# marbl/Mash

Measured on AMD Instinct MI355X. Metric: pairwise Mash distances/sec (s=1000), higher is better.
Workload: dtype u64; 1 GPU; mash triangle all-vs-all, 100000 clustered synthetic sketches, k=21 s=1000, 4999950000 pairs/step, per-table job (index build + discover + fill + merge each step), row-block sharded x1; parallelism=rowblock1, rccl_ranks=0

## Files before the change

### mash_amd/csrc/compare_dense.hip

```cpp
#ifdef MG_HIP_EMU
#include "hipemu.h"
#else
#include <hip/hip_runtime.h>
#define MG_DYN_SHARED(T, name)                                   \
    extern __shared__ __align__(16) unsigned char name##_raw[]; \
    T *name = reinterpret_cast<T *>(name##_raw)
#endif
#include <stdint.h>

#include <cstdlib>

#ifndef MG_HIP_EMU
#include <rocprim/device/device_radix_sort.hpp>
#include <rocprim/device/device_select.hpp>
#include <rocprim/iterator/counting_iterator.hpp>
#endif

#include "compare_internal.h"

namespace mg {

#ifndef MG_HIP_EMU
__global__ __launch_bounds__(256) void dn_neighbor_kernel(const uint64_t *hashes, uint64_t stride, const uint32_t *cnt, uint32_t n,
                                                          uint8_t *link)
// ... 126 lines not shown
{
    if (E == 0) return hipSuccess;
    hipError_t e = hipMemsetAsync(cnt, 0, DN_SUBLISTS * 4, stream);
    if (e == hipSuccess) e = hipMemsetAsync(total, 0, 8, stream);
    if (e != hipSuccess) return e;
    hipLaunchKernelGGL(dn_leaders_kernel, dim3((E + 255u) / 256u), dim3(256), 0, stream, sorted_rows, gs_of, gend, grp_of, groups, E, key, val, cap_sub,
                       cnt);
    e = hipGetLastError();
    if (e != hipSuccess) return e;
    return dense_join_leaders(key, val, cap_sub, key_out, val_out, cnt, off, total, stream);
}

hipError_t dense_join_leaders(const unsigned long long *key, const uint32_t *val, uint32_t cap_sub, unsigned long long *key_out, uint32_t *val_out,
                              const uint32_t *cnt, uint32_t *off, uint32_t *total, hipStream_t stream)
{
    hipLaunchKernelGGL(dn_sublists_scan_kernel, dim3(1), dim3(DN_SUBLISTS), 0, stream, cnt, cap_sub, off, total);
    hipLaunchKernelGGL(dn_sublists_copy_kernel, dim3(DN_SUBLISTS), dim3(256), 0, stream, key, val, cnt, (const uint32_t *)off, cap_sub, key_out, val_out);
    return hipGetLastError();
}

hipError_t dense_sort_universes(const unsigned long long *key, const uint32_t *val, uint32_t m, void *temp, size_t temp_bytes,
                                unsigned long long *key_sorted, uint32_t *ulist, uint32_t *upos, uint32_t *ustart, uint32_t *uend,
                                uint32_t group_bits, hipStream_t stream)
{
    if (m == 0) return hipSuccess;
    hipError_t e = rocprim::radix_sort_pairs(temp, temp_bytes, key, key_sorted, val, upos, (size_t)m, 0u, 32u + group_bits, stream);
    if (e != hipSuccess) return e;
    hipLaunchKernelGGL(dn_universe_split_kernel, dim3((m + 255u) / 256u), dim3(256), 0, stream, (const unsigned long long *)key_sorted, m, ulist,
                       ustart, uend);
    return hipGetLastError();
}

#endif

constexpr uint32_t DN_CX_MASK = 0x7FFFu, DN_CX_FLAG = 0x8000u;

template <uint32_t DN_EK>
__global__ __launch_bounds__(256) void dn_encode_kernel(const uint32_t *off, const uint32_t *code_img, uint32_t *pos_img, uint32_t rs,
                                                        const uint32_t *grp_of, const DenseGroup *groups, const uint32_t *ulist,
                                                        const uint32_t *upos, unsigned long long *gdata, uint32_t wstride, uint16_t *ext,
                                                        uint32_t xs, uint32_t n, uint32_t ul_in_lds)
{
    MG_DYN_SHARED(uint32_t, lds);
    const uint32_t bid = blockIdx.x;
    const uint32_t row = (bid & ~63u) | ((bid & 7u) << 3) | ((bid >> 3) & 7u);
    const uint32_t tid = threadIdx.x, lane = tid & 63u, wid = tid >> 6;
    if (row >= n) return;
    const uint32_t g = grp_of[row];
    if (g == 0xFFFFFFFFu) return;
    const DenseGroup G = groups[g];
    const uint32_t W = G.W, u = G.u;
    uint32_t *mask32 = lds, *hist = lds + 2u * W, *gap8 = hist + W + 1u, *ovf = gap8 + 16u * W, *pl32 = ovf + W, *scr = pl32 + 8u * W;
    uint32_t *ull = lds + 28u * wstride + 9u;
    for (uint32_t i = tid; i < 28u * W + 1u; i += 256u) lds[i] = 0;
    const uint32_t *ulg = ulist + G.ustart, *up = upos + G.ustart;
    if (ul_in_lds)
        for (uint32_t i = tid; i < u; i += 256u) ull[i] = ulg[i];
    const uint32_t *ul = ul_in_lds ? ull : ulg;
    __syncthreads();
    const uint32_t cnt = off[row + 1] - off[row];
    uint16_t *xrow = ext + (uint64_t)(G.xrow0 + (row - G.g0)) * xs;
    uint32_t nx = 0;
    if constexpr (DN_EK == 1) {
        for (uint32_t base = 0; base < cnt; base += 256u) {
            const uint32_t p = base + tid;
            uint32_t idx = 0;
// ... 493 lines not shown
{
    const uint32_t a = blockIdx.x;
    const uint64_t *src = hashes + (uint64_t)inv[a] * stride;
    uint64_t *dst = out + (uint64_t)a * stride;
    for (uint64_t p = threadIdx.x; p < stride; p += 256u) dst[p] = src[p];
}

hipError_t launch_dense_gather_rows(const uint64_t *hashes, uint64_t stride, const uint32_t *inv, uint32_t n, uint64_t *out, hipStream_t stream)
{
    if (n == 0) return hipSuccess;
    hipLaunchKernelGGL(cl_gather_rows_kernel, dim3(n), dim3(256), 0, stream, hashes, stride, inv, out);
    return hipGetLastError();
}

#endif

__global__ __launch_bounds__(256) void dn_group_rows_kernel(const DenseGroup *groups, uint32_t ng, uint32_t n, uint32_t *grp_of, uint4 *lead_rows)
{
    const uint32_t r = blockIdx.x * 256u + threadIdx.x;
    if (r >= n) return;
    uint32_t lo = 0, hi = ng;
    while (lo < hi) {
        const uint32_t mid = (lo + hi) >> 1;
        if (groups[mid].g0 <= r) lo = mid + 1u;
        else hi = mid;
    }
    uint32_t g = 0xFFFFFFFFu, g0 = 0, g1 = 0;
    if (lo > 0 && r < groups[lo - 1u].g1) {
        g = lo - 1u;
        g0 = groups[g].g0;
        g1 = groups[g].g1;
    }
    grp_of[r] = g;
    lead_rows[r] = make_uint4(g, g0, g1, 0u);
}

hipError_t launch_dense_group_rows(const DenseGroup *groups, uint32_t ng, uint32_t n, uint32_t *grp_of, uint32_t *lead_rows, hipStream_t stream)
{
    if (n == 0) return hipSuccess;
    hipLaunchKernelGGL(dn_group_rows_kernel, dim3((n + 255u) / 256u), dim3(256), 0, stream, groups, ng, n, grp_of, reinterpret_cast<uint4 *>(lead_rows));
    return hipGetLastError();
}

}
```

### mash_amd/csrc/compare_internal.h

```cpp
#pragma once
#ifdef MG_HIP_EMU
#include "hipemu.h"
#else
#include <hip/hip_runtime.h>
#endif
#include <stdint.h>

namespace mg {

struct MergedTile {
    uint32_t rows[32];
    uint32_t col0, col1;
};

struct CompareArgs {
    const uint64_t *row_hashes;
    const uint32_t *row_nhash;
    const uint64_t *col_hashes;
    const uint32_t *col_nhash;
    const uint32_t *row_pfx;
    const uint32_t *col_pfx;
    const MergedTile *mtiles;
    uint2 *out;
    uint64_t row_stride, col_stride;
// ... 137 lines not shown
    uint32_t g0, g1;
    uint32_t ustart, u;
    uint32_t W;
    uint32_t xrow0;
    uint64_t data_off;
};
struct DenseTile { uint32_t group, row0, cblk; };
#ifdef __HIPCC__
__host__ __device__
#endif
static inline uint64_t dense_block_planes(uint32_t W) { return 128ull * W + 64ull * (W + 1u); }
#ifdef __HIPCC__
__host__ __device__
#endif
static inline uint64_t dense_block_words(uint32_t W) { return dense_block_planes(W) + 512ull * W; }
struct DenseList {
    const uint32_t *row_base = nullptr, *row_cnt = nullptr;
    uint2 *rc = nullptr, *counts = nullptr;
    uint32_t row_first = 0;
};
hipError_t launch_dense_neighbors(const uint64_t *hashes, uint64_t stride, const uint32_t *cnt, uint32_t n, uint8_t *link,
                                  hipStream_t stream);
size_t dense_universe_temp_bytes(uint32_t cap);
uint32_t dense_sublists();
hipError_t dense_find_leaders(const uint32_t *sorted_rows, const uint32_t *gs_of, const uint32_t *gend, const uint32_t *grp_of,
                              const DenseGroup *groups, uint32_t E, unsigned long long *key, uint32_t *val, uint32_t cap_sub,
                              unsigned long long *key_out, uint32_t *val_out, uint32_t *cnt, uint32_t *off, uint32_t *total,
                              hipStream_t stream);
hipError_t dense_join_leaders(const unsigned long long *key, const uint32_t *val, uint32_t cap_sub, unsigned long long *key_out, uint32_t *val_out,
                              const uint32_t *cnt, uint32_t *off, uint32_t *total, hipStream_t stream);
hipError_t dense_sort_universes(const unsigned long long *key, const uint32_t *val, uint32_t m, void *temp, size_t temp_bytes,
                                unsigned long long *key_sorted, uint32_t *ulist, uint32_t *upos, uint32_t *ustart, uint32_t *uend,
                                uint32_t group_bits, hipStream_t stream);
hipError_t launch_dense_encode(const uint32_t *off, const uint32_t *code_img, uint32_t *pos_img, uint32_t rs, const uint32_t *grp_of,
                               const DenseGroup *groups, const uint32_t *ulist, const uint32_t *upos, unsigned long long *gdata,
                               uint16_t *ext, uint32_t xs, uint32_t n, uint32_t wmax, hipStream_t stream, int ul_mode = -1);
size_t dense_pairs_lds(uint32_t W, uint32_t rows);
uint32_t dense_rows_per_tile(uint64_t wave_rows);
uint32_t dense_max_words();
hipError_t launch_dense_pairs(const DenseTile *tiles, uint32_t ntiles, uint32_t rows_per_tile, const DenseGroup *groups,
                              const unsigned long long *gdata, bool use_lists, const uint16_t *ext, uint32_t xs,
                              uint32_t s, uint32_t wmax, uint32_t row_begin, uint32_t row_end, uint64_t out_base, const uint32_t *inv, uint2 *out,
                              hipStream_t stream, const DenseList *list = nullptr);
size_t dense_cluster_temp_bytes(uint32_t n);
hipError_t dense_cluster_rows(const uint64_t *hashes, uint64_t stride, const uint32_t *cnt, uint32_t n, void *temp, size_t temp_bytes,
                              unsigned long long *key_a, unsigned long long *key_b, uint32_t *row_a, uint32_t *row_b, uint32_t *lab_a,
                              uint32_t *lab_b, uint32_t *inv, uint32_t *label_sorted, hipStream_t stream, uint32_t split = 0);
hipError_t launch_dense_gather_rows(const uint64_t *hashes, uint64_t stride, const uint32_t *inv, uint32_t n, uint64_t *out, hipStream_t stream);
hipError_t launch_dense_group_rows(const DenseGroup *groups, uint32_t ng, uint32_t n, uint32_t *grp_of, uint32_t *lead_rows, hipStream_t stream);

struct JoinSide {
    const uint2 *grp = nullptr;
    const uint32_t *ent = nullptr;
    const uint32_t *goff = nullptr;
    const uint32_t *gend = nullptr;
    const uint32_t *thr = nullptr;
};
struct JoinArgs {
    JoinSide rows, cols;
    const uint32_t *row_cnt_off, *col_cnt_off;
    const uint32_t *rep, *col_rep;
    const uint32_t *inv;
    uint2 *out;
    uint64_t out_base;
    uint64_t ntiles;
    uint32_t ncols;
// ... 41 lines not shown
```

### mash_amd/csrc/host_index.cpp

```cpp
#include "host_internal.h"
#include "index_build.h"
#ifdef IX_PHASE_CLOCKS
namespace mg { void index_dump_clocks(); }
#endif
#include "sort_bits.h"

namespace {

const uint64_t kTilesLongestRun = 6144;
static const uint64_t kSplitMinRun = 128;

uint64_t longest_label_run(const uint32_t *lab_sorted, uint64_t n)
{
    if (!lab_sorted || n == 0) return 0;
    uint64_t run = 1, longest = 1;
    for (uint64_t a = 1; a < n; a++) {
        run = lab_sorted[a] == lab_sorted[a - 1] ? run + 1 : 1;
        longest = std::max(longest, run);
    }
    return longest;
}

struct Carve {
    unsigned char *base = nullptr;
    size_t at = 0;
    template <class T> T *take(size_t count)
    {
        const size_t from = (at + alignof(T) - 1) & ~(alignof(T) - 1);
        at = from + count * sizeof(T);
        return base ? reinterpret_cast<T *>(base + from) : nullptr;
    }
};

struct LeaderLists {
    DevBuf<unsigned long long> key, keyj;
    DevBuf<uint32_t> val, valj, cnt_sub, off_sub, nlead;
    uint32_t lists = mg::dense_sublists(), cap = 0, tot[2] = {0, 0};
    explicit LeaderLists(mg_ctx *c) : key(c), keyj(c), val(c), valj(c), cnt_sub(c), off_sub(c), nlead(c) {}

    hipError_t alloc(uint32_t room)
    {
        key.free(); val.free(); keyj.free(); valj.free();
        const uint64_t all = (uint64_t)lists * room;
        if (!(nlead.p && cnt_sub.p && off_sub.p) && (nlead.alloc(2) != hipSuccess || cnt_sub.alloc(lists) != hipSuccess || off_sub.alloc(lists) != hipSuccess))
            return hipErrorOutOfMemory;
        if (key.alloc(all) != hipSuccess || val.alloc(all) != hipSuccess || keyj.alloc(all) != hipSuccess || valj.alloc(all) != hipSuccess) return hipErrorOutOfMemory;
        cap = room;
        return hipSuccess;
    }
    hipError_t reset(hipStream_t st) { const hipError_t e = hipMemsetAsync(cnt_sub, 0, lists * 4, st); return e != hipSuccess ? e : hipMemsetAsync(nlead, 0, 8, st); }
    hipError_t join(hipStream_t st)
    {
        const hipError_t e = mg::dense_join_leaders(key, val, cap, keyj, valj, cnt_sub, off_sub, nlead, st);
        return e != hipSuccess ? e : hipMemcpyAsync(tot, nlead, 8, hipMemcpyDeviceToHost, st);
    }
    mg::IxLeaders view(const uint32_t *lead_rows) const { return mg::IxLeaders{lead_rows, key, val, cnt_sub, cap, lists}; }
    bool overflowed() const { return tot[1] > cap; }
};

struct SparseIndexBuild {
    mg_ctx *ctx;
    const mg_table *t;
    const uint32_t s;
    const bool clustered;
    const uint32_t split;
    mg_table::Sparse *sp;
    const uint64_t n;
    const std::chrono::steady_clock::time_point t_begin = std::chrono::steady_clock::now();
    bool stop = false;

    bool need_classes = false, dedup = true, want_dense = true, try_cluster = false, try_links = false;
    DevBuf<uint8_t> dc_cls, d_link;
    DevBuf<unsigned long long> dc_last, d_dig, d_dig_sorted, k_a, k_b;
    DevBuf<uint32_t> d_cnt, d_rows_sorted, d_flags, d_nflag, r_a, r_b, l_a, l_b, d_inv, d_lab;
    DevBuf<unsigned char> d_tmp_dup, d_tmp_cl;
    std::vector<uint8_t> hc_cls, link;
    std::vector<uint64_t> hc_last;
    std::vector<uint32_t> hc_nh, inv_v, lab_v;
    const uint32_t *inv = nullptr, *lab_sorted = nullptr;
    uint32_t nflag = 0;
    size_t tb_dup = 0, tb_cl = 0;
    bool cluster_q = false, links_q = false;

    const char *ix_mode = nullptr;
    bool ix_verify = false, ix_tiles = true;
    std::vector<uint32_t> cnt_true, cnt_perm;
    uint32_t max_cnt = 0;
    uint64_t maxv = 0, E_all = 0;
    double dens[65] = {0};
    double dens0 = 0;
    std::vector<uint32_t> rep;
    const uint64_t *H = nullptr;
    mg::IxPlan early_plan;
    DevBuf<unsigned char> d_lb;
    bool lb_made = false;
    bool cnt_stale = false;

    std::vector<uint32_t> cls_of, cls_off, cls_rows, cls_first;

    uint32_t E = 0, end_bit = 0, sort_begin_bit = 0;
    std::vector<mg::DenseGroup> cand_groups;
    std::vector<uint32_t> grp_of_h;
    DevBuf<mg::DenseGroup> d_groups;
    DevBuf<uint32_t> d_grp_of, d_lead_rows;
    LeaderLists lead;
    bool lead_ready = false, cand_prepared = false;
    mg::IxPlan plan;
    size_t temp_bytes = 0;
    DevBuf<unsigned char> temp;
    DevBuf<uint32_t> gs_of;
    DevBuf<unsigned long long> key64_a, key64_b;
    struct Stat { unsigned long long shared; uint32_t max_group, groups, bad, tie_overflow; uint32_t ixf[4]; } h_stat = {0, 0, 0, 0, 0, {0, 0, 0, 0}};
    DevBuf<Stat> d_stat;
    DevBuf<unsigned char> d_slots;
    bool want_order = true;
    std::vector<uint32_t> short_cnt;

    bool built = false;
    uint64_t dn_xrows = 0, dn_words = 0;

    SparseIndexBuild(mg_ctx *c, const mg_table *tab, uint32_t sketch_size, bool clustered_variant, mg_table::Sparse *index, uint32_t split_row)
        : ctx(c), t(tab), s(sketch_size), clustered(clustered_variant), split(split_row), sp(index), n(tab->n), dc_cls(c), d_link(c), dc_last(c), d_dig(c), d_dig_sorted(c),
          k_a(c), k_b(c), d_cnt(c), d_rows_sorted(c), d_flags(c), d_nflag(c), r_a(c), r_b(c), l_a(c), l_b(c), d_inv(c), d_lab(c), d_tmp_dup(c), d_tmp_cl(c), d_lb(c),
          d_groups(c), d_grp_of(c), d_lead_rows(c), lead(c), temp(c), gs_of(c), key64_a(c), key64_b(c), d_stat(c), d_slots(c)
    {}

    int unusable(const char *why) { sp->usable = false; sp->why = why; stop = true; return MG_OK; }

    hipError_t counts_to_device()
    {
            if (!cnt_stale) return hipSuccess;
            cnt_stale = false;
            return hipMemcpyAsync(d_cnt, cnt_true.data(), n * 4, hipMemcpyHostToDevice, ctx->stream);
    }

    template <class T> bool take(T **p, size_t count)
    {
        void *q = nullptr;
        if (ctx_malloc(ctx, &q, std::max<size_t>(count, 1) * sizeof(T)) != hipSuccess) return false;
        *p = static_cast<T *>(q);
        return true;
    }

    void drop()
    {
            for (void **q : {(void **)&sp->off, (void **)&sp->keys_sorted, (void **)&sp->gend, (void **)&sp->sorted_rows, (void **)&sp->code_img,
                             (void **)&sp->pos_img, (void **)&sp->short_rows, (void **)&sp->short_cnt, (void **)&sp->counters, (void **)&sp->order,
                             (void **)&sp->rep, (void **)&sp->cls_of, (void **)&sp->cls_off, (void **)&sp->cls_rows, (void **)&sp->cls_first})
                if (*q) { ctx_free(ctx, *q); *q = nullptr; }
    }

    int no_memory() { (void)hipGetLastError(); drop(); return unusable("no device memory for the index"); }
    int lost(hipError_t e) { drop(); return fail(ctx, MG_ERR_HIP, std::string("compare (index build): ") + hipGetErrorString(e)); }

    void drop_dense()
    {
        for (void **q : {(void **)&sp->dgroups, (void **)&sp->grp_of, (void **)&sp->gdata, (void **)&sp->ext, (void **)&sp->ulist, (void **)&sp->upos})
            if (*q) { ctx_free(ctx, *q); *q = nullptr; }
        sp->dgroups_host.clear();
    }

    struct TileScratch {
        DevBuf<unsigned char> tcnt, start, big, pk, tc;
        explicit TileScratch(mg_ctx *c) : tcnt(c), start(c), big(c), pk(c), tc(c) {}
    };

    hipError_t tiles(const TileScratch &w, int stages)
    {
        const mg::IxLeaders lv = lead.view(d_lead_rows);
        return mg::index_build(plan, H, sp->off, d_lb, w.tcnt, w.start, w.big, w.pk, w.tc, sp->keys_sorted, sp->sorted_rows, sp->gend, gs_of, sp->code_img,
                               sp->pos_img, d_slots, &d_stat.p->shared, &d_stat.p->max_group, &d_stat.p->groups, d_stat.p->ixf, lead_ready ? &lv : nullptr,
                               ctx->stream, stages);
    }
    hipError_t sort_buckets(const TileScratch &w)
    {
        hipError_t e = tiles(w, 2);
        if (e == hipSuccess && lead_ready) e = lead.join(ctx->stream);
        return e != hipSuccess ? e : hipMemcpyAsync(&h_stat, d_stat, sizeof(Stat), hipMemcpyDeviceToHost, ctx->stream);
    }
    hipError_t row_order()
    {
        return mg::launch_sparse_row_order(sp->off, sp->code_img, sp->gend, sp->rep, (uint32_t)n, sp->rs, temp, temp_bytes, key64_a, key64_b, sp->order, ctx->stream);
    }

    int scan_rows();
    int order_rows();
    int find_copies();
    int lay_out();
    void prepare_candidates();
    hipError_t tile_passes();
    int build_by_tiles();
    int build_by_sort();
    int check_build();
    bool search_leaders();
    bool sort_universes(std::vector<uint32_t> &us, std::vector<uint32_t> &ue);
    bool choose_groups(const std::vector<uint32_t> &us, const std::vector<uint32_t> &ue);
    int encode_groups();
    int dense_groups();
    int run();
};

int SparseIndexBuild::scan_rows()
{
    need_classes = t->cls.size() != n;
    dedup = !ctx_opt(ctx, "MASHGPU_SPARSE_NO_DEDUP");
    want_dense = true;
    if (const char *v = ctx_opt(ctx, "MASHGPU_COMPARE_DENSE")) want_dense = atoi(v) != 0;
    try_cluster = clustered && n >= 16;
    try_links = !try_cluster && want_dense && n >= 8 && s <= 16384;
    tb_dup = mg::sparse_dup_temp_bytes((uint32_t)n);
    tb_cl = mg::dense_cluster_temp_bytes((uint32_t)n);
    if (d_cnt.alloc(n) != hipSuccess || (need_classes && (dc_cls.alloc(n) != hipSuccess || dc_last.alloc(n) != hipSuccess)) ||
        (dedup && (d_dig.alloc(n) != hipSuccess || d_dig_sorted.alloc(n) != hipSuccess || d_rows_sorted.alloc(n) != hipSuccess ||
                   d_flags.alloc(n) != hipSuccess || d_nflag.alloc(1) != hipSuccess || d_tmp_dup.alloc(std::max<size_t>(tb_dup, 16)) != hipSuccess))) {
        (void)hipGetLastError();
        return unusable("no device memory for the index");
    }
    {
        hipError_t e = hipSuccess;
        if (need_classes) {
            hc_cls.resize(n);
            hc_last.resize(n);
            hc_nh.resize(n);
            e = mg::launch_row_classes(t->hashes, t->nhash, n, t->s, dc_cls, dc_last, ctx->stream);
        }
        if (e == hipSuccess) e = mg::launch_sparse_row_counts(t->nhash, (uint32_t)n, (uint32_t)std::min<uint64_t>(t->s, s), d_cnt, ctx->stream);
        if (e == hipSuccess && dedup) {
            e = mg::launch_sparse_row_digest(t->hashes, t->s, d_cnt, (uint32_t)n, d_dig, ctx->stream);
            if (e == hipSuccess)
                e = mg::launch_sparse_dup_suspects(d_dig, d_cnt, (uint32_t)n, d_tmp_dup, tb_dup, d_dig_sorted, d_rows_sorted, d_flags, d_nflag, ctx->stream);
        }
        if (e == hipSuccess && try_cluster) {
            if (k_a.alloc(4 * n) == hipSuccess && k_b.alloc(4 * n) == hipSuccess && r_a.alloc(4 * n) == hipSuccess && r_b.alloc(4 * n) == hipSuccess &&
                l_a.alloc(n) == hipSuccess && l_b.alloc(n) == hipSuccess && d_inv.alloc(n) == hipSuccess && d_lab.alloc(n) == hipSuccess &&
                d_tmp_cl.alloc(std::max<size_t>(tb_cl, 16)) == hipSuccess) {
                e = mg::dense_cluster_rows(t->hashes, t->s, d_cnt, (uint32_t)n, d_tmp_cl, tb_cl, k_a, k_b, r_a, r_b, l_a, l_b, d_inv, d_lab, ctx->stream, split);
                cluster_q = true;
            } else {
                (void)hipGetLastError();
            }
        }
        if (e == hipSuccess && try_links) {
            if (d_link.alloc(n) == hipSuccess) {
                link.resize(n);
                e = mg::launch_dense_neighbors(t->hashes, t->s, d_cnt, (uint32_t)n, d_link, ctx->stream);
                links_q = true;
            } else {
                (void)hipGetLastError();
            }
        }
        unsigned long long *p_last = nullptr;
        uint32_t *p_nh = nullptr, *p_inv = nullptr, *p_lab = nullptr, *p_nflag = nullptr;
        uint8_t *p_cls = nullptr, *p_link = nullptr;
        auto carve = [&](unsigned char *block) {
            Carve c{block};
            p_last = c.take<unsigned long long>(n); p_nh = c.take<uint32_t>(n); p_inv = c.take<uint32_t>(n); p_lab = c.take<uint32_t>(n);
            p_nflag = c.take<uint32_t>(2); p_cls = c.take<uint8_t>(n); p_link = c.take<uint8_t>(n);
            return c.at + 64;
        };
        unsigned char *pin = static_cast<unsigned char *>(ctx_pinned(ctx, carve(nullptr)));
        if (pin) {
            carve(pin);
        } else {
            p_nflag = &nflag;
            if (cluster_q) { inv_v.resize(n); lab_v.resize(n); p_inv = inv_v.data(); p_lab = lab_v.data(); }
            p_nh = hc_nh.data(); p_cls = hc_cls.data(); p_last = reinterpret_cast<unsigned long long *>(hc_last.data()); p_link = link.data();
        }
        if (e == hipSuccess && need_classes) {
            e = hipMemcpyAsync(p_nh, t->nhash, n * 4, hipMemcpyDeviceToHost, ctx->stream);
            if (e == hipSuccess) e = hipMemcpyAsync(p_cls, dc_cls, n, hipMemcpyDeviceToHost, ctx->stream);
            if (e == hipSuccess) e = hipMemcpyAsync(p_last, dc_last, n * 8, hipMemcpyDeviceToHost, ctx->stream);
        }
        if (e == hipSuccess && dedup) e = hipMemcpyAsync(p_nflag, d_nflag, 4, hipMemcpyDeviceToHost, ctx->stream);
        if (e == hipSuccess && cluster_q) {
            e = hipMemcpyAsync(p_inv, d_inv, n * 4, hipMemcpyDeviceToHost, ctx->stream);
            if (e == hipSuccess) e = hipMemcpyAsync(p_lab, d_lab, n * 4, hipMemcpyDeviceToHost, ctx->stream);
        }
        if (e == hipSuccess && links_q) e = hipMemcpyAsync(p_link, d_link, n, hipMemcpyDeviceToHost, ctx->stream);
        const hipError_t es = hipStreamSynchronize(ctx->stream);
        if (e == hipSuccess) e = es;
        if (e == hipSuccess && pin) {
            if (need_classes) {
                memcpy(hc_nh.data(), p_nh, n * 4);
                memcpy(hc_cls.data(), p_cls, n);
                memcpy(hc_last.data(), p_last, n * 8);
            }
            if (dedup) nflag = *p_nflag;
            if (links_q) memcpy(link.data(), p_link, n);
        }
        if (cluster_q) { inv = p_inv; lab_sorted = p_lab; }
        if (e != hipSuccess) return fail(ctx, MG_ERR_HIP, std::string("compare (index: rows, copies, order): ") + hipGetErrorString(e));
    }
    if (need_classes) {
        t->cls.swap(hc_cls);
        t->last.swap(hc_last);
        t->nh.swap(hc_nh);
// ... 185 lines not shown
        if (e == hipSuccess && !v.empty()) e = hipMemcpyAsync(dst, v.data(), v.size() * 4, hipMemcpyHostToDevice, ctx->stream);
    };
    if (sp->copies) { upload(sp->rep, rep); upload(sp->cls_of, cls_of); upload(sp->cls_off, cls_off); upload(sp->cls_rows, cls_rows); upload(sp->cls_first, cls_first); }
    if (!rep.empty()) upload(sp->off, sp->off_host);
    else if (e == hipSuccess) e = mg::launch_sparse_offsets(d_cnt, cnt_stale ? sp->inv : nullptr, (uint32_t)n, temp, sp->off, ctx->stream);
    upload(sp->short_rows, sp->short_rows_host); upload(sp->short_cnt, short_cnt);
    return e == hipSuccess ? MG_OK : lost(e);
}

void SparseIndexBuild::prepare_candidates()
{
    if (cand_prepared) return;
    cand_prepared = true;
    if (link.empty() || sp->copies != 0) return;
    for (uint64_t i = 1; i < n;) {
        if (!link[i]) { i++; continue; }
        uint64_t j = i;
        while (j < n && link[j]) j++;
        if (j - (i - 1) >= 8) {
            mg::DenseGroup g{};
            g.g0 = (uint32_t)(i - 1); g.g1 = (uint32_t)j;
            cand_groups.push_back(g);
        }
        i = j + 1;
    }
    if (cand_groups.empty()) return;
    const uint32_t ng = (uint32_t)cand_groups.size();
    grp_of_h.assign(n, 0xFFFFFFFFu);
    for (uint32_t g = 0; g < ng; g++)
        for (uint32_t r = cand_groups[g].g0; r < cand_groups[g].g1; r++) grp_of_h[r] = g;
    uint32_t room = std::max<uint32_t>(E / 4u / lead.lists + 64u, 256u);
    if (const char *ev = ctx_opt(ctx, "MASHGPU_DENSE_LEAD_CAP")) room = std::max<uint32_t>((uint32_t)atoi(ev), 1u);
    if (d_groups.alloc(ng) == hipSuccess && d_grp_of.alloc(n) == hipSuccess && d_lead_rows.alloc(4 * n) == hipSuccess && lead.alloc(room) == hipSuccess &&
        hipMemcpyAsync(d_groups, cand_groups.data(), ng * sizeof(mg::DenseGroup), hipMemcpyHostToDevice, ctx->stream) == hipSuccess &&
        mg::launch_dense_group_rows(d_groups, ng, (uint32_t)n, d_grp_of, d_lead_rows, ctx->stream) == hipSuccess && lead.reset(ctx->stream) == hipSuccess) {
        lead_ready = true;
    } else {
        (void)hipGetLastError();
        cand_groups.clear();
    }
}

hipError_t SparseIndexBuild::tile_passes()
{
    TileScratch w(ctx);
    if (!((lb_made || d_lb.alloc(plan.lb_bytes) == hipSuccess) && w.tcnt.alloc(plan.cnt_bytes) == hipSuccess && w.start.alloc(plan.start_bytes) == hipSuccess &&
          w.big.alloc(plan.big_bytes) == hipSuccess && w.pk.alloc(plan.pk_bytes) == hipSuccess && w.tc.alloc(plan.tc_bytes) == hipSuccess)) {
        (void)hipGetLastError();
        return hipSuccess;
    }
    hipError_t e = hipMemsetAsync(d_stat, 0, sizeof(Stat), ctx->stream);
    if (e == hipSuccess) e = tiles(w, lb_made ? 1 | 8 : 1);
    DevBuf<uint32_t> d_swapped(ctx);
    if (e == hipSuccess && ctx_opt(ctx, "MASHGPU_IX_DEBUG_SWAP") && d_swapped.alloc(1) == hipSuccess) {
        e = hipMemsetAsync(d_swapped, 0, 4, ctx->stream);
        if (e == hipSuccess) e = mg::index_debug_swap(plan, w.pk, w.start, d_swapped, ctx->stream);
    }
    if (e == hipSuccess) prepare_candidates();
    if (e == hipSuccess && ctx->aside_at_sort) ctx->aside_at_sort();
    if (e == hipSuccess) e = sort_buckets(w);
    hipEvent_t ev_stats = nullptr;
    if (e == hipSuccess) e = hipEventCreateWithFlags(&ev_stats, hipEventDisableTiming);
    if (e == hipSuccess) e = hipEventRecord(ev_stats, ctx->stream);
    if (e == hipSuccess) e = tiles(w, 4);
    if (e == hipSuccess && want_order) e = row_order();
    const hipError_t ew = e == hipSuccess ? hipEventSynchronize(ev_stats) : hipStreamSynchronize(ctx->stream);
    if (e == hipSuccess) e = ew;
    if (ev_stats) (void)hipEventDestroy(ev_stats);
    built = e == hipSuccess && !h_stat.ixf[mg::IXF_DEGENERATE];
    if (built && lead_ready && lead.overflowed() && h_stat.ixf[mg::IXF_NBIG] == 0) {
        e = hipStreamSynchronize(ctx->stream);
        const uint32_t want_cap = lead.tot[1];
        if (e == hipSuccess && lead.alloc(want_cap) == hipSuccess) {
            e = lead.reset(ctx->stream);
            if (e == hipSuccess) e = hipMemsetAsync(d_stat.p, 0, offsetof(Stat, bad), ctx->stream);
            if (e == hipSuccess) e = sort_buckets(w);
            if (e == hipSuccess) e = hipStreamSynchronize(ctx->stream);
            built = e == hipSuccess && !h_stat.ixf[mg::IXF_DEGENERATE];
            if (ctx_opt(ctx, "MASHGPU_SPARSE_DBG"))
                fprintf(stderr, "compare dense: a list of leaders asked for %u entries: found again with that room (%u leaders)\n", want_cap, lead.tot[0]);
        } else {
            (void)hipGetLastError();
        }
    }
    if (ctx_opt(ctx, "MASHGPU_SPARSE_DBG"))
        fprintf(stderr, "compare sparse: index by tiles: shift %u, %u buckets (%u per window, %u windows), fullest %u, %u beyond the LDS (%u values streamed)%s\n",
                plan.g.shift, plan.g.Bp, plan.g.BW, plan.g.NW, h_stat.ixf[mg::IXF_MAXBUCKET], h_stat.ixf[mg::IXF_NBIG], h_stat.ixf[mg::IXF_NSTREAMED],
                h_stat.ixf[mg::IXF_DEGENERATE] ? " -- clumped values: sorted instead" : "");
    return e;
}

int SparseIndexBuild::build_by_tiles()
{
    hipError_t e = hipSuccess;
    if (plan.ok) e = tile_passes();
    else if (ix_tiles && ctx_opt(ctx, "MASHGPU_SPARSE_DBG")) fprintf(stderr, "compare sparse: index by tiles refused: %s\n", plan.why);
    if (e != hipSuccess) return lost(e);
    sp->by_tiles = built;
    prepare_candidates();
#ifdef IX_PHASE_CLOCKS
    if (built && ctx_opt(ctx, "MASHGPU_IX_CLOCKS")) mg::index_dump_clocks();
#endif
    if (ix_verify && !built && !ctx_opt(ctx, "MASHGPU_SPARSE_INDEX_MAY_REFUSE"))
        return fail(ctx, MG_ERR_INVALID, std::string("index verify: the tile build refused this table (") + (plan.ok ? "bucket flags" : plan.why) + ")");
    return MG_OK;
}

int SparseIndexBuild::build_by_sort()
{
    if (built && !ix_verify) return MG_OK;
// ... 44 lines not shown
    if (e != hipSuccess) return lost(e);
    std::string msg;
    for (int k = 0; k < 6; k++)
        if (diff[2 * k]) msg += std::string(msg.empty() ? "" : "; ") + arrays[k].name + ": " + std::to_string(diff[2 * k]) + " differ, first at " + std::to_string(diff[2 * k + 1]);
    if (h_stat.shared != tiles_stat.shared || h_stat.max_group != tiles_stat.max_group || h_stat.groups != tiles_stat.groups)
        msg += std::string(msg.empty() ? "" : "; ") + "statistics: shared " + std::to_string(tiles_stat.shared) + " / " + std::to_string(h_stat.shared) +
               ", largest group " + std::to_string(tiles_stat.max_group) + " / " + std::to_string(h_stat.max_group) + ", groups " +
               std::to_string(tiles_stat.groups) + " / " + std::to_string(h_stat.groups);
    if (!msg.empty()) {
        char geom[160];
        snprintf(geom, sizeof geom, " [n %llu, E %u, shift %u, %u buckets, %u per window, %u windows]", (unsigned long long)n, E, plan.g.shift, plan.g.Bp, plan.g.BW, plan.g.NW);
        sp->usable = false;
        return fail(ctx, MG_ERR_INVALID, "index verify: tiles / sort -- " + msg + geom);
    }
    return MG_OK;
}

int SparseIndexBuild::check_build()
{
    if (h_stat.bad) { drop(); return unusable("sort order inside a value not by row"); }
    sp->G = h_stat.groups;
    sp->shared = h_stat.shared;
    sp->max_group = h_stat.max_group;
    sp->build_ms = std::chrono::duration<double, std::milli>(std::chrono::steady_clock::now() - t_begin).count();
    sp->usable = true;
    return MG_OK;
}

bool SparseIndexBuild::search_leaders()
{
    for (int attempt = 0;; attempt++) {
        hipError_t e = mg::dense_find_leaders(sp->sorted_rows, gs_of, sp->gend, d_grp_of, d_groups, E, lead.key, lead.val, lead.cap, lead.keyj, lead.valj,
                                              lead.cnt_sub, lead.off_sub, lead.nlead, ctx->stream);
        if (e == hipSuccess) e = hipMemcpyAsync(lead.tot, lead.nlead, 8, hipMemcpyDeviceToHost, ctx->stream);
        if (e == hipSuccess) e = hipStreamSynchronize(ctx->stream);
        if (e != hipSuccess) return false;
        if (!lead.overflowed() || attempt >= 1) return true;
        if (lead.alloc(lead.tot[1]) != hipSuccess) return false;
    }
}

bool SparseIndexBuild::sort_universes(std::vector<uint32_t> &us, std::vector<uint32_t> &ue)
{
    const uint32_t ng = (uint32_t)cand_groups.size(), nlead = lead.tot[0];
    uint32_t gbits = 1;
    while ((1u << gbits) < ng) gbits++;
    const size_t tb = mg::dense_universe_temp_bytes(nlead);
    DevBuf<uint32_t> d_us(ctx), d_ue(ctx);
    DevBuf<unsigned long long> d_key2(ctx);
    DevBuf<unsigned char> d_utmp(ctx);
    bool ok = d_us.alloc(ng) == hipSuccess && d_ue.alloc(ng) == hipSuccess && d_key2.alloc(nlead) == hipSuccess && d_utmp.alloc(std::max<size_t>(tb, 16)) == hipSuccess;
    if (!ok || !take(&sp->ulist, nlead) || !take(&sp->upos, nlead)) return false;
    hipError_t e = hipMemsetAsync(d_us, 0, ng * 4, ctx->stream);
    if (e == hipSuccess) e = hipMemsetAsync(d_ue, 0, ng * 4, ctx->stream);
    if (e == hipSuccess) e = mg::dense_sort_universes(lead.keyj, lead.valj, nlead, d_utmp, tb, d_key2, sp->ulist, sp->upos, d_us, d_ue, gbits, ctx->stream);
    if (e == hipSuccess) e = hipMemcpyAsync(us.data(), d_us, ng * 4, hipMemcpyDeviceToHost, ctx->stream);
    if (e == hipSuccess) e = hipMemcpyAsync(ue.data(), d_ue, ng * 4, hipMemcpyDeviceToHost, ctx->stream);
    if (e == hipSuccess) e = hipStreamSynchronize(ctx->stream);
    return e == hipSuccess;
}

bool SparseIndexBuild::choose_groups(const std::vector<uint32_t> &us, const std::vector<uint32_t> &ue)
{
    const uint32_t kMaxWords = mg::dense_max_words();
    std::fill(grp_of_h.begin(), grp_of_h.end(), 0xFFFFFFFFu);
    for (uint32_t g = 0; g < (uint32_t)cand_groups.size(); g++) {
        mg::DenseGroup G = cand_groups[g];
        G.u = ue[g] > us[g] ? ue[g] - us[g] : 0u;
        G.ustart = us[g];
        G.W = (G.u >> 6) + 1u;
        if (G.u < 32u || G.W > kMaxWords) continue;
        G.xrow0 = (uint32_t)dn_xrows;
        G.data_off = dn_words;
        const uint64_t m = G.g1 - G.g0;
        dn_xrows += m;
        dn_words += ((m + 127) / 128) * mg::dense_block_words(G.W);
        sp->dn_wmax = std::max(sp->dn_wmax, G.W);
        for (uint32_t r = G.g0; r < G.g1; r++) grp_of_h[r] = (uint32_t)sp->dgroups_host.size();
        sp->dgroups_host.push_back(G);
    }
    return !sp->dgroups_host.empty();
}

int SparseIndexBuild::encode_groups()
{
    sp->dn_xs = ((s + 7u) & ~7u) + 8u;
    if (!take(&sp->dgroups, sp->dgroups_host.size()) || !take(&sp->grp_of, n) || !take(&sp->gdata, dn_words) || !take(&sp->ext, dn_xrows * sp->dn_xs)) {
        (void)hipGetLastError();
        sp->dgroups_host.clear();
        return MG_OK;
    }
    hipError_t e = hipMemcpyAsync(sp->dgroups, sp->dgroups_host.data(), sp->dgroups_host.size() * sizeof(mg::DenseGroup), hipMemcpyHostToDevice, ctx->stream);
    if (e == hipSuccess) e = hipMemcpyAsync(sp->grp_of, grp_of_h.data(), n * 4, hipMemcpyHostToDevice, ctx->stream);
    if (e == hipSuccess)
        e = mg::launch_dense_encode(sp->off, sp->code_img, sp->pos_img, sp->rs, sp->grp_of, sp->dgroups, sp->ulist, sp->upos, sp->gdata, sp->ext, sp->dn_xs,
                                    (uint32_t)n, sp->dn_wmax, ctx->stream, ctx_opt(ctx, "MASHGPU_DENSE_UL_LDS") ? atoi(ctx_opt(ctx, "MASHGPU_DENSE_UL_LDS")) : -1);
    sp->grp_of_host.swap(grp_of_h);
    if (e != hipSuccess) {
        drop();
        drop_dense();
        sp->usable = false;
        return fail(ctx, MG_ERR_HIP, std::string("compare (index build, dense groups): ") + hipGetErrorString(e));
    }
    sp->dn_lists = ctx_opt(ctx, "MASHGPU_DENSE_LISTS") != nullptr;
    return MG_OK;
}

int SparseIndexBuild::dense_groups()
{
    if (!cand_groups.empty()) {
        auto t_dense = std::chrono::steady_clock::now();
        if (built && lead_ready && lead.overflowed() && ctx_opt(ctx, "MASHGPU_SPARSE_DBG"))
            fprintf(stderr, "compare dense: a list of leaders asked for %u entries, room for %u: no dense groups for this table\n", lead.tot[1], lead.cap);
        std::vector<uint32_t> us(cand_groups.size(), 0), ue(cand_groups.size(), 0);
        const int rc = [&] {
            if (!lead_ready || (!built && !search_leaders())) return (int)MG_OK;
            if (lead.tot[0] == 0 || lead.overflowed()) return (int)MG_OK;
            return sort_universes(us, ue) && choose_groups(us, ue) ? encode_groups() : (int)MG_OK;
        }();
        if (rc != MG_OK) return rc;
        if (sp->dgroups_host.empty()) { (void)hipGetLastError(); drop_dense(); }
        sp->build_ms += std::chrono::duration<double, std::milli>(std::chrono::steady_clock::now() - t_dense).count();
        if (ctx_opt(ctx, "MASHGPU_SPARSE_DBG")) {
            uint64_t rows_in = 0;
            for (auto &G : sp->dgroups_host) rows_in += G.g1 - G.g0;
            fprintf(stderr, "compare dense: %zu chains of related rows, %zu groups kept (%llu rows, widest universe %u words)\n", cand_groups.size(),
                    sp->dgroups_host.size(), (unsigned long long)rows_in, sp->dn_wmax);
        }
    }
    if (ctx_opt(ctx, "MASHGPU_SPARSE_DBG"))
        fprintf(stderr, "compare sparse: index of %llu rows (%llu copies of earlier rows), s %u: %u entries, %u distinct, shared %llu, largest run %u, %.2f ms\n",
                (unsigned long long)n, (unsigned long long)sp->copies, s, E, sp->G, (unsigned long long)sp->shared, sp->max_group, sp->build_ms);
    return MG_OK;
}

int SparseIndexBuild::run()
{
    int rc = MG_OK;
    if ((rc = scan_rows()) != MG_OK || stop) return rc;
    if ((rc = order_rows()) != MG_OK || stop) return rc;
    if ((rc = find_copies()) != MG_OK || stop) return rc;
    if ((rc = lay_out()) != MG_OK || stop) return rc;
    if ((rc = build_by_tiles()) != MG_OK || stop) return rc;
    if ((rc = build_by_sort()) != MG_OK || stop) return rc;
    if ((rc = check_build()) != MG_OK || stop) return rc;
    return dense_groups();
}

}

int table_sparse_index(mg_ctx *ctx, const mg_table *t, uint32_t s, bool clustered, mg_table::Sparse **out, uint32_t split)
// ... 23 lines not shown
```

Baseline: 432.9 billion pairs/s.

## Replace global radix sort of dense universes with per-group counting and LDS bitonic sort

Adds a counting pass that builds a per-chunk, per-group histogram and a prefix scan, so universe start and end offsets are known once leaders are joined. The counts are copied back with the existing stats readback, which avoids the separate sort-and-split round trip. Entries are then scattered into group segments and each group is bitonic-sorted in LDS. Group rows are now assigned on the GPU instead of uploading grp_of from the host, and pinned staging is used for groups. If any universe exceeds the LDS capacity, or there are too many groups, it falls back to the old radix sort path.

```diff
diff --git a/mash_amd/csrc/compare_dense.hip b/mash_amd/csrc/compare_dense.hip
--- a/mash_amd/csrc/compare_dense.hip
+++ b/mash_amd/csrc/compare_dense.hip
@@ -182,6 +182,150 @@
 }
 
 #endif
+
+constexpr uint32_t DN_USORT_CAP = 16384, DN_USORT_THREADS = 1024, DN_UCHUNKS = 128, DN_UGROUPS_MAX = 16384;
+
+__global__ __launch_bounds__(DN_USORT_THREADS) void dn_group_count_kernel(const unsigned long long *key, const uint32_t *nlead, uint32_t ng, uint32_t *mat)
+{
+    MG_DYN_SHARED(uint32_t, hist);
+    const uint32_t m = nlead[0], chunk = (m + DN_UCHUNKS - 1u) / DN_UCHUNKS, t = threadIdx.x;
+    const uint32_t from = blockIdx.x * chunk < m ? blockIdx.x * chunk : m, to = m - from < chunk ? m : from + chunk;
+    for (uint32_t g = t; g < ng; g += DN_USORT_THREADS) hist[g] = 0;
+    __syncthreads();
+    for (uint32_t i = from + t; i < to; i += DN_USORT_THREADS) {
+        const uint32_t g = (uint32_t)(key[i] >> 32);
+        if (g < ng) atomicAdd(&hist[g], 1u);
+    }
+    __syncthreads();
+    for (uint32_t g = t; g < ng; g += DN_USORT_THREADS) mat[(size_t)blockIdx.x * ng + g] = hist[g];
+}
+
+__global__ __launch_bounds__(DN_USORT_THREADS) void dn_group_scan_kernel(uint32_t *mat, uint32_t ng, uint32_t *us, uint32_t *ue)
+{
+    __shared__ uint32_t s_w[DN_USORT_THREADS / 64];
+    const uint32_t t = threadIdx.x, lane = t & 63u, wid = t >> 6;
+    uint32_t carry = 0;
+    for (uint32_t base = 0; base < ng; base += DN_USORT_THREADS) {
+        const uint32_t g = base + t;
+        uint32_t c = 0;
+        if (g < ng)
+            for (uint32_t b = 0; b < DN_UCHUNKS; b++) c += mat[(size_t)b * ng + g];
+        uint32_t incl = c;
+#pragma unroll
+        for (uint32_t d = 1; d < 64u; d <<= 1) {
+            const uint32_t x = __shfl_up(incl, d);
+            if (lane >= d) incl += x;
+        }
+        if (lane == 63u) s_w[wid] = incl;
+        __syncthreads();
+        uint32_t before = 0, all = 0;
+        for (uint32_t k = 0; k < DN_USORT_THREADS / 64u; k++) {
+            before += k < wid ? s_w[k] : 0u;
+            all += s_w[k];
+        }
+        uint32_t at = carry + before + incl - c;
+        if (g < ng) {
+            us[g] = c ? at : 0u;
+            ue[g] = c ? at + c : 0u;
+            for (uint32_t b = 0; b < DN_UCHUNKS; b++) {
+                const uint32_t x = mat[(size_t)b * ng + g];
+                mat[(size_t)b * ng + g] = at;
+                at += x;
+            }
+        }
+        carry += all;
+        __syncthreads();
+    }
+}
+
+__global__ __launch_bounds__(DN_USORT_THREADS) void dn_universe_scatter_kernel(const unsigned long long *key, const uint32_t *val, uint32_t m, uint32_t ng,
+                                                                               const uint32_t *mat, unsigned long long *seg)
+{
+    MG_DYN_SHARED(uint32_t, cursor);
+    const uint32_t chunk = (m + DN_UCHUNKS - 1u) / DN_UCHUNKS, t = threadIdx.x;
+    const uint32_t from = blockIdx.x * chunk < m ? blockIdx.x * chunk : m, to = m - from < chunk ? m : from + chunk;
+    for (uint32_t g = t; g < ng; g += DN_USORT_THREADS) cursor[g] = mat[(size_t)blockIdx.x * ng + g];
+    __syncthreads();
+    for (uint32_t i = from + t; i < to; i += DN_USORT_THREADS) {
+        const unsigned long long k = key[i];
+        const uint32_t g = (uint32_t)(k >> 32);
+        if (g >= ng) continue;
+        const uint32_t slot = atomicAdd(&cursor[g], 1u);
+        if (slot < m) seg[slot] = (k << 32) | val[i];
+    }
+}
+
+__global__ __launch_bounds__(DN_USORT_THREADS) void dn_universe_sort_kernel(const unsigned long long *seg, const uint32_t *us, const uint32_t *ue,
+                                                                            uint32_t m, uint32_t *ulist, uint32_t *upos)
+{
+    MG_DYN_SHARED(unsigned long long, srt);
+    const uint32_t g = blockIdx.x, t = threadIdx.x;
+    const uint32_t a = us[g], b = ue[g];
+    if (b <= a || b > m || b - a > DN_USORT_CAP) return;
+    const uint32_t u = b - a;
+    uint32_t P = 1;
+    while (P < u) P <<= 1;
+    for (uint32_t i = t; i < P; i += DN_USORT_THREADS) srt[i] = i < u ? seg[a + i] : ~0ull;
+    __syncthreads();
+    for (uint32_t k = 2; k <= P; k <<= 1)
+        for (uint32_t j = k >> 1; j > 0; j >>= 1) {
+            for (uint32_t i = t; i < (P >> 1); i += DN_USORT_THREADS) {
+                const uint32_t lo = ((i & ~(j - 1u)) << 1) | (i & (j - 1u)), hi = lo | j;
+                const unsigned long long x = srt[lo], y = srt[hi];
+                if ((x > y) == ((lo & k) == 0u)) {
+                    srt[lo] = y;
+                    srt[hi] = x;
+                }
+            }
+            __syncthreads();
+        }
+    for (uint32_t i = t; i < u; i += DN_USORT_THREADS) {
+        const unsigned long long x = srt[i];
+        ulist[a + i] = (uint32_t)(x >> 32);
+        upos[a + i] = (uint32_t)x;
+    }
+}
+
+uint32_t dense_universe_lds_capacity() { return DN_USORT_CAP; }
+uint32_t dense_universe_max_groups() { return DN_UGROUPS_MAX; }
+size_t dense_universe_matrix_words(uint32_t ngroups) { return (size_t)DN_UCHUNKS * ngroups; }
+
+hipError_t dense_count_universes(const unsigned long long *key, const uint32_t *nlead, uint32_t ngroups, uint32_t *mat, uint32_t *us, uint32_t *ue,
+                                 hipStream_t stream)
+{
+    if (ngroups > DN_UGROUPS_MAX) return hipErrorInvalidValue;
+    if (ngroups == 0) return hipSuccess;
+    const size_t smem = (size_t)ngroups * 4;
+    const hipError_t e = hipFuncSetAttribute(reinterpret_cast<const void *>(dn_group_count_kernel), hipFuncAttributeMaxDynamicSharedMemorySize, (int)smem);
+    if (e != hipSuccess) return e;
+    hipLaunchKernelGGL(dn_group_count_kernel, dim3(DN_UCHUNKS), dim3(DN_USORT_THREADS), smem, stream, key, nlead, ngroups, mat);
+    hipLaunchKernelGGL(dn_group_scan_kernel, dim3(1), dim3(DN_USORT_THREADS), 0, stream, mat, ngroups, us, ue);
+    return hipGetLastError();
+}
+
+bool dense_universes_fit_lds(const uint32_t *us, const uint32_t *ue, uint32_t ngroups, uint32_t *max_u)
+{
+    uint32_t mx = 0;
+    for (uint32_t g = 0; g < ngroups; g++) mx = ue[g] > us[g] && ue[g] - us[g] > mx ? ue[g] - us[g] : mx;
+    if (max_u) *max_u = mx;
+    return mx <= DN_USORT_CAP;
+}
+
+hipError_t dense_group_universes(const unsigned long long *key, const uint32_t *val, uint32_t m, uint32_t ngroups, const uint32_t *mat, const uint32_t *us,
+                                 const uint32_t *ue, uint32_t max_u, unsigned long long *seg, uint32_t *ulist, uint32_t *upos, hipStream_t stream)
+{
+    if (max_u > DN_USORT_CAP || ngroups > DN_UGROUPS_MAX) return hipErrorInvalidValue;
+    if (m == 0 || ngroups == 0) return hipSuccess;
+    uint32_t P = 1;
+    while (P < max_u) P <<= 1;
+    const size_t smem = (size_t)P * 8, smem_sc = (size_t)ngroups * 4;
+    hipError_t e = hipFuncSetAttribute(reinterpret_cast<const void *>(dn_universe_sort_kernel), hipFuncAttributeMaxDynamicSharedMemorySize, (int)smem);
+    if (e == hipSuccess) e = hipFuncSetAttribute(reinterpret_cast<const void *>(dn_universe_scatter_kernel), hipFuncAttributeMaxDynamicSharedMemorySize, (int)smem_sc);
+    if (e != hipSuccess) return e;
+    hipLaunchKernelGGL(dn_universe_scatter_kernel, dim3(DN_UCHUNKS), dim3(DN_USORT_THREADS), smem_sc, stream, key, val, m, ngroups, mat, seg);
+    hipLaunchKernelGGL(dn_universe_sort_kernel, dim3(ngroups), dim3(DN_USORT_THREADS), smem, stream, (const unsigned long long *)seg, us, ue, m, ulist, upos);
+    return hipGetLastError();
+}
 
 constexpr uint32_t DN_CX_MASK = 0x7FFFu, DN_CX_FLAG = 0x8000u;
 
@@ -741,7 +885,7 @@
         g1 = groups[g].g1;
     }
     grp_of[r] = g;
-    lead_rows[r] = make_uint4(g, g0, g1, 0u);
+    if (lead_rows) lead_rows[r] = make_uint4(g, g0, g1, 0u);
 }
 
 hipError_t launch_dense_group_rows(const DenseGroup *groups, uint32_t ng, uint32_t n, uint32_t *grp_of, uint32_t *lead_rows, hipStream_t stream)
diff --git a/mash_amd/csrc/compare_internal.h b/mash_amd/csrc/compare_internal.h
--- a/mash_amd/csrc/compare_internal.h
+++ b/mash_amd/csrc/compare_internal.h
@@ -193,6 +193,14 @@
 hipError_t dense_sort_universes(const unsigned long long *key, const uint32_t *val, uint32_t m, void *temp, size_t temp_bytes,
                                 unsigned long long *key_sorted, uint32_t *ulist, uint32_t *upos, uint32_t *ustart, uint32_t *uend,
                                 uint32_t group_bits, hipStream_t stream);
+uint32_t dense_universe_lds_capacity();
+uint32_t dense_universe_max_groups();
+size_t dense_universe_matrix_words(uint32_t ngroups);
+hipError_t dense_count_universes(const unsigned long long *key, const uint32_t *nlead, uint32_t ngroups, uint32_t *mat, uint32_t *us, uint32_t *ue,
+                                 hipStream_t stream);
+bool dense_universes_fit_lds(const uint32_t *us, const uint32_t *ue, uint32_t ngroups, uint32_t *max_u);
+hipError_t dense_group_universes(const unsigned long long *key, const uint32_t *val, uint32_t m, uint32_t ngroups, const uint32_t *mat, const uint32_t *us,
+                                 const uint32_t *ue, uint32_t max_u, unsigned long long *seg, uint32_t *ulist, uint32_t *upos, hipStream_t stream);
 hipError_t launch_dense_encode(const uint32_t *off, const uint32_t *code_img, uint32_t *pos_img, uint32_t rs, const uint32_t *grp_of,
                                const DenseGroup *groups, const uint32_t *ulist, const uint32_t *upos, unsigned long long *gdata,
                                uint16_t *ext, uint32_t xs, uint32_t n, uint32_t wmax, hipStream_t stream, int ul_mode = -1);
diff --git a/mash_amd/csrc/host_index.cpp b/mash_amd/csrc/host_index.cpp
--- a/mash_amd/csrc/host_index.cpp
+++ b/mash_amd/csrc/host_index.cpp
@@ -49,11 +49,8 @@
         return hipSuccess;
     }
     hipError_t reset(hipStream_t st) { const hipError_t e = hipMemsetAsync(cnt_sub, 0, lists * 4, st); return e != hipSuccess ? e : hipMemsetAsync(nlead, 0, 8, st); }
-    hipError_t join(hipStream_t st)
-    {
-        const hipError_t e = mg::dense_join_leaders(key, val, cap, keyj, valj, cnt_sub, off_sub, nlead, st);
-        return e != hipSuccess ? e : hipMemcpyAsync(tot, nlead, 8, hipMemcpyDeviceToHost, st);
-    }
+    hipError_t join(hipStream_t st) { return mg::dense_join_leaders(key, val, cap, keyj, valj, cnt_sub, off_sub, nlead, st); }
+    hipError_t totals_back(hipStream_t st) { return hipMemcpyAsync(tot, nlead, 8, hipMemcpyDeviceToHost, st); }
     mg::IxLeaders view(const uint32_t *lead_rows) const { return mg::IxLeaders{lead_rows, key, val, cnt_sub, cap, lists}; }
     bool overflowed() const { return tot[1] > cap; }
 };
@@ -104,6 +101,12 @@
     DevBuf<mg::DenseGroup> d_groups;
     DevBuf<uint32_t> d_grp_of, d_lead_rows;
     LeaderLists lead;
+    DevBuf<uint32_t> d_use, d_umat;
+    bool counted = false;
+    uint32_t *pin_use = nullptr;
+    mg::DenseGroup *pin_groups = nullptr;
+    const uint32_t *use_h = nullptr;
+    std::vector<uint32_t> use_v;
     bool lead_ready = false, cand_prepared = false;
     mg::IxPlan plan;
     size_t temp_bytes = 0;
@@ -122,7 +125,7 @@
     SparseIndexBuild(mg_ctx *c, const mg_table *tab, uint32_t sketch_size, bool clustered_variant, mg_table::Sparse *index, uint32_t split_row)
         : ctx(c), t(tab), s(sketch_size), clustered(clustered_variant), split(split_row), sp(index), n(tab->n), dc_cls(c), d_link(c), dc_last(c), d_dig(c), d_dig_sorted(c),
           k_a(c), k_b(c), d_cnt(c), d_rows_sorted(c), d_flags(c), d_nflag(c), r_a(c), r_b(c), l_a(c), l_b(c), d_inv(c), d_lab(c), d_tmp_dup(c), d_tmp_cl(c), d_lb(c),
-          d_groups(c), d_grp_of(c), d_lead_rows(c), lead(c), temp(c), gs_of(c), key64_a(c), key64_b(c), d_stat(c), d_slots(c)
+          d_groups(c), d_grp_of(c), d_lead_rows(c), lead(c), d_use(c), d_umat(c), temp(c), gs_of(c), key64_a(c), key64_b(c), d_stat(c), d_slots(c)
     {}
 
     int unusable(const char *why) { sp->usable = false; sp->why = why; stop = true; return MG_OK; }
@@ -175,8 +178,29 @@
     hipError_t sort_buckets(const TileScratch &w)
     {
         hipError_t e = tiles(w, 2);
-        if (e == hipSuccess && lead_ready) e = lead.join(ctx->stream);
+        if (e == hipSuccess && lead_ready) e = join_leaders();
         return e != hipSuccess ? e : hipMemcpyAsync(&h_stat, d_stat, sizeof(Stat), hipMemcpyDeviceToHost, ctx->stream);
+    }
+    hipError_t join_leaders()
+    {
+        const hipError_t e = lead.join(ctx->stream);
+        return e != hipSuccess ? e : count_universes();
+    }
+    hipError_t count_universes()
+    {
+        const uint32_t ng = (uint32_t)cand_groups.size();
+        hipError_t e = counted ? mg::dense_count_universes(lead.keyj, lead.nlead, ng, d_umat, d_use, d_use.p + ng, ctx->stream) : hipSuccess;
+        if (e == hipSuccess && counted && pin_use) e = hipMemcpyAsync(pin_use, d_use, (size_t)ng * 8, hipMemcpyDeviceToHost, ctx->stream);
+        return e != hipSuccess ? e : lead.totals_back(ctx->stream);
+    }
+    hipError_t universes_back()
+    {
+        if (!counted) return hipSuccess;
+        if (pin_use) { use_h = pin_use; return hipSuccess; }
+        use_v.resize(2 * cand_groups.size());
+        use_h = use_v.data();
+        const hipError_t e = hipMemcpyAsync(use_v.data(), d_use, use_v.size() * 4, hipMemcpyDeviceToHost, ctx->stream);
+        return e != hipSuccess ? e : hipStreamSynchronize(ctx->stream);
     }
     hipError_t row_order()
     {
@@ -194,7 +218,8 @@
     int check_build();
     bool search_leaders();
     bool sort_universes(std::vector<uint32_t> &us, std::vector<uint32_t> &ue);
-    bool choose_groups(const std::vector<uint32_t> &us, const std::vector<uint32_t> &ue);
+    bool group_universes(uint32_t max_u);
+    bool choose_groups(const uint32_t *us, const uint32_t *ue);
     int encode_groups();
     int dense_groups();
     int run();
@@ -256,12 +281,14 @@
             Carve c{block};
             p_last = c.take<unsigned long long>(n); p_nh = c.take<uint32_t>(n); p_inv = c.take<uint32_t>(n); p_lab = c.take<uint32_t>(n);
             p_nflag = c.take<uint32_t>(2); p_cls = c.take<uint8_t>(n); p_link = c.take<uint8_t>(n);
+            pin_use = c.take<uint32_t>(2 * (n / 8 + 1)); pin_groups = c.take<mg::DenseGroup>(n / 8 + 1);
             return c.at + 64;
         };
         unsigned char *pin = static_cast<unsigned char *>(ctx_pinned(ctx, carve(nullptr)));
         if (pin) {
             carve(pin);
         } else {
+            pin_use = nullptr; pin_groups = nullptr;
             p_nflag = &nflag;
             if (cluster_q) { inv_v.resize(n); lab_v.resize(n); p_inv = inv_v.data(); p_lab = lab_v.data(); }
             p_nh = hc_nh.data(); p_cls = hc_cls.data(); p_last = reinterpret_cast<unsigned long long *>(hc_last.data()); p_link = link.data();
@@ -513,9 +540,11 @@
     uint32_t room = std::max<uint32_t>(E / 4u / lead.lists + 64u, 256u);
     if (const char *ev = ctx_opt(ctx, "MASHGPU_DENSE_LEAD_CAP")) room = std::max<uint32_t>((uint32_t)atoi(ev), 1u);
     if (d_groups.alloc(ng) == hipSuccess && d_grp_of.alloc(n) == hipSuccess && d_lead_rows.alloc(4 * n) == hipSuccess && lead.alloc(room) == hipSuccess &&
+        d_use.alloc(2 * (size_t)ng) == hipSuccess && (ng > mg::dense_universe_max_groups() || d_umat.alloc(mg::dense_universe_matrix_words(ng)) == hipSuccess) &&
         hipMemcpyAsync(d_groups, cand_groups.data(), ng * sizeof(mg::DenseGroup), hipMemcpyHostToDevice, ctx->stream) == hipSuccess &&
         mg::launch_dense_group_rows(d_groups, ng, (uint32_t)n, d_grp_of, d_lead_rows, ctx->stream) == hipSuccess && lead.reset(ctx->stream) == hipSuccess) {
         lead_ready = true;
+        counted = ng <= mg::dense_universe_max_groups();
     } else {
         (void)hipGetLastError();
         cand_groups.clear();
@@ -548,6 +577,7 @@
     const hipError_t ew = e == hipSuccess ? hipEventSynchronize(ev_stats) : hipStreamSynchronize(ctx->stream);
     if (e == hipSuccess) e = ew;
     if (ev_stats) (void)hipEventDestroy(ev_stats);
+    if (e == hipSuccess && lead_ready) e = universes_back();
     built = e == hipSuccess && !h_stat.ixf[mg::IXF_DEGENERATE];
     if (built && lead_ready && lead.overflowed() && h_stat.ixf[mg::IXF_NBIG] == 0) {
         e = hipStreamSynchronize(ctx->stream);
@@ -557,6 +587,7 @@
             if (e == hipSuccess) e = hipMemsetAsync(d_stat.p, 0, offsetof(Stat, bad), ctx->stream);
             if (e == hipSuccess) e = sort_buckets(w);
             if (e == hipSuccess) e = hipStreamSynchronize(ctx->stream);
+            if (e == hipSuccess) e = universes_back();
             built = e == hipSuccess && !h_stat.ixf[mg::IXF_DEGENERATE];
             if (ctx_opt(ctx, "MASHGPU_SPARSE_DBG"))
                 fprintf(stderr, "compare dense: a list of leaders asked for %u entries: found again with that room (%u leaders)\n", want_cap, lead.tot[0]);
@@ -667,8 +698,9 @@
     for (int attempt = 0;; attempt++) {
         hipError_t e = mg::dense_find_leaders(sp->sorted_rows, gs_of, sp->gend, d_grp_of, d_groups, E, lead.key, lead.val, lead.cap, lead.keyj, lead.valj,
                                               lead.cnt_sub, lead.off_sub, lead.nlead, ctx->stream);
-        if (e == hipSuccess) e = hipMemcpyAsync(lead.tot, lead.nlead, 8, hipMemcpyDeviceToHost, ctx->stream);
+        if (e == hipSuccess) e = count_universes();
         if (e == hipSuccess) e = hipStreamSynchronize(ctx->stream);
+        if (e == hipSuccess) e = universes_back();
         if (e != hipSuccess) return false;
         if (!lead.overflowed() || attempt >= 1) return true;
         if (lead.alloc(lead.tot[1]) != hipSuccess) return false;
@@ -695,7 +727,15 @@
     return e == hipSuccess;
 }
 
-bool SparseIndexBuild::choose_groups(const std::vector<uint32_t> &us, const std::vector<uint32_t> &ue)
+bool SparseIndexBuild::group_universes(uint32_t max_u)
+{
+    const uint32_t ng = (uint32_t)cand_groups.size(), nlead = lead.tot[0];
+    DevBuf<unsigned long long> d_seg(ctx);
+    if (d_seg.alloc(nlead) != hipSuccess || !take(&sp->ulist, nlead) || !take(&sp->upos, nlead)) return false;
+    return mg::dense_group_universes(lead.keyj, lead.valj, nlead, ng, d_umat, d_use, d_use.p + ng, max_u, d_seg, sp->ulist, sp->upos, ctx->stream) == hipSuccess;
+}
+
+bool SparseIndexBuild::choose_groups(const uint32_t *us, const uint32_t *ue)
 {
     const uint32_t kMaxWords = mg::dense_max_words();
     std::fill(grp_of_h.begin(), grp_of_h.end(), 0xFFFFFFFFu);
@@ -725,8 +765,11 @@
         sp->dgroups_host.clear();
         return MG_OK;
     }
-    hipError_t e = hipMemcpyAsync(sp->dgroups, sp->dgroups_host.data(), sp->dgroups_host.size() * sizeof(mg::DenseGroup), hipMemcpyHostToDevice, ctx->stream);
-    if (e == hipSuccess) e = hipMemcpyAsync(sp->grp_of, grp_of_h.data(), n * 4, hipMemcpyHostToDevice, ctx->stream);
+    const size_t nkept = sp->dgroups_host.size();
+    const mg::DenseGroup *src = sp->dgroups_host.data();
+    if (pin_groups) { memcpy(pin_groups, src, nkept * sizeof(mg::DenseGroup)); src = pin_groups; }
+    hipError_t e = hipMemcpyAsync(sp->dgroups, src, nkept * sizeof(mg::DenseGroup), hipMemcpyHostToDevice, ctx->stream);
+    if (e == hipSuccess) e = mg::launch_dense_group_rows(sp->dgroups, (uint32_t)nkept, (uint32_t)n, sp->grp_of, nullptr, ctx->stream);
     if (e == hipSuccess)
         e = mg::launch_dense_encode(sp->off, sp->code_img, sp->pos_img, sp->rs, sp->grp_of, sp->dgroups, sp->ulist, sp->upos, sp->gdata, sp->ext, sp->dn_xs,
                                     (uint32_t)n, sp->dn_wmax, ctx->stream, ctx_opt(ctx, "MASHGPU_DENSE_UL_LDS") ? atoi(ctx_opt(ctx, "MASHGPU_DENSE_UL_LDS")) : -1);
@@ -747,11 +790,17 @@
         auto t_dense = std::chrono::steady_clock::now();
         if (built && lead_ready && lead.overflowed() && ctx_opt(ctx, "MASHGPU_SPARSE_DBG"))
             fprintf(stderr, "compare dense: a list of leaders asked for %u entries, room for %u: no dense groups for this table\n", lead.tot[1], lead.cap);
-        std::vector<uint32_t> us(cand_groups.size(), 0), ue(cand_groups.size(), 0);
+        const uint32_t ng = (uint32_t)cand_groups.size();
         const int rc = [&] {
             if (!lead_ready || (!built && !search_leaders())) return (int)MG_OK;
             if (lead.tot[0] == 0 || lead.overflowed()) return (int)MG_OK;
-            return sort_universes(us, ue) && choose_groups(us, ue) ? encode_groups() : (int)MG_OK;
+            uint32_t max_u = 0;
+            const char *how = ctx_opt(ctx, "MASHGPU_DENSE_UNIVERSES");
+            if ((how && strcmp(how, "sort") == 0) || !use_h || !mg::dense_universes_fit_lds(use_h, use_h + ng, ng, &max_u)) {
+                std::vector<uint32_t> us(ng, 0), ue(ng, 0);
+                return sort_universes(us, ue) && choose_groups(us.data(), ue.data()) ? encode_groups() : (int)MG_OK;
+            }
+            return choose_groups(use_h, use_h + ng) && group_universes(max_u) ? encode_groups() : (int)MG_OK;
         }();
         if (rc != MG_OK) return rc;
         if (sp->dgroups_host.empty()) { (void)hipGetLastError(); drop_dense(); }
```

Result: no change. 436.5 billion pairs/s (median of 6 runs) (+0.9%).
